# fateshelled/sycl_points

Hardware: AMD Instinct MI355X
Metric: gicp_correspondences_per_sec (higher is better)
Workload: dtype f32

## Files before the change

### include/sycl_points_amd.h

```cpp
#ifndef SYCL_POINTS_AMD_H
#define SYCL_POINTS_AMD_H

#include <stddef.h>
#include <stdint.h>

#ifdef __cplusplus
extern "C" {
#endif

#define SP_OK 0
#define SP_ERR_INVALID_ARGUMENT 1
#define SP_ERR_RUNTIME 2
#define SP_ERR_HIP 3

#define SP_ABI_VERSION 7
int sp_abi_version(void);
void sp_stream_retired(void* stream);
const char* sp_last_error(void);

int sp_device_count(void);
int sp_set_device(int device);


size_t sp_knn_bruteforce_workspace_bytes(size_t nq, size_t nt, size_t k);
// ... 278 lines not shown
typedef struct sp_gicp_target sp_gicp_target;
typedef struct sp_gicp_source sp_gicp_source;
typedef struct sp_gn_params { float lambda, crit_rotation, crit_translation; } sp_gn_params;
enum { SP_SOURCE_ORDER_UNKNOWN = 0, SP_SOURCE_SORT = 1, SP_SOURCE_PRESORTED = 2 };
int sp_gicp_target_create(const sp_grid* grid, const float* tgt_covs, size_t n, void* stream, sp_gicp_target** out);
int sp_gicp_target_update(sp_gicp_target* target, const float* tgt_covs, void* stream);
int sp_gicp_target_create_plain(const sp_grid* grid, const float* tgt_covs, size_t n, void* stream, sp_gicp_target** out);
int sp_gicp_target_certify(sp_gicp_target* target, const float* tgt_covs, void* stream);
int sp_gicp_target_has_certificates(const sp_gicp_target* target);
int sp_gicp_target_prepare(sp_gicp_target* target, const float* tgt_covs, int reg_type, void* stream);
void sp_gicp_target_destroy(sp_gicp_target* target);
int sp_gicp_source_create(size_t n_max, sp_gicp_source** out);
int sp_gicp_source_prepare(sp_gicp_source* source, const sp_gicp_target* target, const float* src_points,
                           const float* src_covs, size_t n, const float* transT, int transT_on_device, int sort_by_cell,
                           void* stream);
void sp_gicp_source_destroy(sp_gicp_source* source);
int sp_gicp_iteration_fused(const sp_gicp_target* target, const sp_gicp_source* source, float* transT,
                            int transT_on_device, const sp_factor_params* params, const sp_gn_params* gn,
                            int32_t* nn_idx_out, float* nn_d2_out, sp_linearized* out, float* delta_out8,
                            void* workspace, size_t workspace_bytes, void* stream);
int sp_gicp_error_prepared(const sp_gicp_target* target, const sp_gicp_source* source, const float* transT_lin_host,
                           const float* transT_trial, int trial_on_device, const sp_factor_params* params,
                           sp_linearized* out, void* workspace, size_t workspace_bytes, void* stream);
int sp_gicp_align_fused(const sp_gicp_target* target, const sp_gicp_source* source, float* transT_device,
                        const sp_factor_params* params, const sp_gn_params* gn, int max_iterations,
                        int32_t* nn_idx_out, float* nn_d2_out, sp_linearized* lin_out, float* delta_out8,
                        uint32_t* iterations_out, void* workspace, size_t workspace_bytes, void* stream);
int sp_gicp_align_step(const sp_gicp_target* target, const sp_gicp_source* source, float* transT_device,
                       const sp_factor_params* params, const sp_gn_params* gn, int k, int rows_all_reduced,
                       int32_t* nn_idx_out, float* nn_d2_out, sp_linearized* lin_out, void* workspace,
// ... 361 lines not shown
```

### sycl_points_amd/_lib.py

```python
import ctypes as C
import os
import subprocess

_HERE = os.path.dirname(os.path.abspath(__file__))
LIB_PATH = os.environ.get("SP_AMD_LIB") or os.path.join(_HERE, "lib", "libsycl_points_amd.so")
CSRC = os.path.join(_HERE, "csrc")

SP_OK, SP_ERR_INVALID_ARGUMENT, SP_ERR_RUNTIME, SP_ERR_HIP = 0, 1, 2, 3
COMM_ID_BYTES = 128


class SpError(RuntimeError):

    def __init__(self, code, msg):
        super().__init__(f"[sycl_points_amd] error {code}: {msg}")
        self.code = code


class Linearized(C.Structure):
    _fields_ = [("H", C.c_float * 36), ("b", C.c_float * 6), ("error", C.c_float), ("inlier", C.c_uint32),
                ("inlier_lo", C.c_float), ("inlier_hi", C.c_float), ("pad", C.c_float * 2)]


class FactorParams(C.Structure):
# ... 250 lines not shown
    "sp_gicp_workspace_bytes": (_sz, [_sz]),
    "sp_gicp_linearize": (_i, [_vp, _vp, _sz, _vp, _vp, _vp, _vp, _vp, _vp, _i, C.POINTER(FactorParams), _vp, _vp, _sz, _vp]),
    "sp_gicp_error": (_i, [_vp, _vp, _sz, _vp, _vp, _vp, _vp, _vp, _vp, _i, C.POINTER(FactorParams), _vp, _vp, _sz, _vp]),
    "sp_icp_robust_weights": (_i, [_vp, _vp, _sz, _vp, _vp, _vp, _vp, _vp, _vp, _i, C.POINTER(FactorParams), _vp, _vp]),
    "sp_genz_counts": (_i, [_vp, _vp, _vp, _sz, _f, _f, _vp, _vp]),
    "sp_gicp_target_create": (_i, [_vp, _vp, _sz, _vp, C.POINTER(_vp)]),
    "sp_gicp_target_create_plain": (_i, [_vp, _vp, _sz, _vp, C.POINTER(_vp)]),
    "sp_gicp_target_certify": (_i, [_vp, _vp, _vp]),
    "sp_gicp_target_has_certificates": (_i, [_vp]),
    "sp_gicp_target_update": (_i, [_vp, _vp, _vp]),
    "sp_gicp_target_prepare": (_i, [_vp, _vp, _i, _vp]),
    "sp_gicp_error_prepared": (_i, [_vp, _vp, _vp, _vp, _i, C.POINTER(FactorParams), _vp, _vp, _sz, _vp]),
    "sp_gicp_target_destroy": (None, [_vp]),
    "sp_gicp_source_create": (_i, [_sz, C.POINTER(_vp)]),
    "sp_gicp_source_prepare": (_i, [_vp, _vp, _vp, _vp, _sz, _vp, _i, _i, _vp]),
    "sp_gicp_source_destroy": (None, [_vp]),
    "sp_gicp_iteration_fused": (_i, [_vp, _vp, _vp, _i, C.POINTER(FactorParams), _vp, _vp, _vp, _vp, _vp, _vp, _sz, _vp]),
    "sp_gicp_align_optimize": (_i, [_vp, _vp, _vp, C.POINTER(FactorParams), C.POINTER(OptParams), C.POINTER(C.c_float), _i, _vp, _vp,
                                    _sz, _vp]),
    "sp_gicp_source_set_persistent": (_i, [_vp, _i]),
    "sp_gicp_source_set_wave_per_point": (_i, [_vp, _i]),
    "sp_gicp_align_batch_workspace_bytes": (_sz, [_sz, _sz]),
    "sp_gicp_align_batch": (_i, [_vp, _vp, _vp, _vp, _sz, C.POINTER(FactorParams), C.POINTER(OptParams), C.POINTER(C.c_float), _i, _vp,
                                 _vp, _sz, _vp]),
    "sp_align_best_host": (_i, [_vp, _sz, C.POINTER(_sz)]),
    "sp_opt_stepper_create": (_i, [C.POINTER(OptParams), _vp, C.POINTER(C.c_float), _i, C.POINTER(_vp)]),
    "sp_opt_stepper_destroy": (None, [_vp]),
    "sp_opt_stepper_next": (_i, [_vp, C.POINTER(OptRequest)]),
    "sp_opt_stepper_linearized": (_i, [_vp, C.POINTER(Linearized)]),
    "sp_opt_stepper_trial": (_i, [_vp, _f, C.c_uint32, C.POINTER(C.c_float)]),
# ... 96 lines not shown
    "sp_pc2_pack": (_i, [_vp, _vp, _vp, _vp, _sz, C.c_double, _vp, _vp]),
    "sp_enhanced_reflectivity_workspace_bytes": (_sz, [_sz]),
    "sp_enhanced_reflectivity": (_i, [_vp, _vp, _sz, _vp, C.c_uint32, C.c_int32, _i, C.c_int32, _vp, _f, _f, _vp, _vp]),
}


INTERNAL_SIGNATURES = {
    "sp_internal_source_option": (_i, [_vp, _i, _i]),
    "sp_internal_grid_option": (_i, [_vp, _i, _i]),
    "sp_internal_bvh_option": (_i, [_vp, _i, _i]),
    "sp_internal_bvh_walk_counts": (_i, [_vp, C.POINTER(C.c_uint32), C.POINTER(C.c_uint32)]),
    "sp_internal_grid_small_build": (_i, [_i]),
    "sp_internal_align_searched_log": (_vp, [_vp, _vp]),
    "sp_internal_source_tile_floats": (_sz, [_vp]),
    "sp_internal_source_tiles_copy": (_i, [_vp, _vp, _sz, _i, _vp]),
    "sp_internal_radix_sort_workspace_bytes": (_sz, [_sz]),
    "sp_internal_radix_sort_u32": (_i, [_vp, _vp, _vp, _vp, _sz, C.c_uint, _vp, _sz, _vp, _vp]),
    "sp_internal_radix_sort_u32_ex": (_i, [_vp, _vp, _vp, _vp, _sz, C.c_uint, C.c_uint, _i, _vp, _sz, _vp, _vp]),
    "sp_internal_radix_first_pass": (None, [_sz, C.c_uint, _vp]),
    "sp_internal_radix_sort_u64": (_i, [_vp, _vp, _vp, _vp, _sz, C.c_uint, _vp, _sz, _vp, _vp]),
    "sp_internal_exclusive_scan_workspace_bytes": (_sz, [_sz]),
    "sp_internal_exclusive_scan_u32": (_i, [_vp, _vp, _sz, _vp, _vp, _sz, _vp]),
    "sp_internal_atan2f_host": (None, [_vp, _vp, _sz, _vp]),
    "sp_internal_fps": (_i, [_i, _vp, _sz, _sz, C.c_uint32, _vp, _vp, _vp, _vp, _sz, _vp]),
    "sp_internal_eigen3": (_i, [_vp, _sz, _vp, _vp, _vp]),
    "sp_internal_inverse3": (_i, [_vp, _sz, _vp, _vp]),
    "sp_internal_bbox": (_i, [_vp, _sz, C.c_uint, _vp, _vp]),
    "sp_internal_morton_keys": (_i, [_vp, _sz, _vp, _vp, _i, _vp, _vp]),
    "sp_internal_sorted_insert": (_i, [_i, _i, _i, _vp, _vp, _sz, _sz, _vp, _vp, _vp]),
    "sp_internal_block_reduce": (_i, [_vp, _vp, _i, _i, _vp, _vp]),
# ... 45 lines not shown
```

### sycl_points_amd/api.py

```python
import ctypes as C
import enum
import sys
import weakref
from dataclasses import dataclass, field

import numpy as np
import torch

from . import _lib
from ._lib import (DegenerateRegParams, FactorParams, GnParams, Linearized, MapPriorParams, MapPriorState, SpError,
                   check)

_SOURCE_ORDER = {False: 0, True: 1, 0: 0, 1: 1, 2: 2, "presorted": 2}
REG = {"POINT_TO_POINT": 0, "POINT_TO_PLANE": 1, "POINT_TO_DISTRIBUTION": 2, "GICP": 3, "GENZ": 4}
LOSS = {"NONE": 0, "HUBER": 1, "TUKEY": 2, "CAUCHY": 3, "GEMAN_MCCLURE": 4}
FLT_MAX = float(np.finfo(np.float32).max)


def _stream():
    return C.c_void_p(torch.cuda.current_stream().cuda_stream)


def _ptr(t):
    return None if t is None else C.c_void_p(t.data_ptr())
# ... 1422 lines not shown
        except Exception:
            pass


class PreparedSource:

    def __init__(self, n_max):
        h = C.c_void_p()
        check(_lib.lib().sp_gicp_source_create(n_max, C.byref(h)))
        self._h = h
        self.n_max = n_max

    def _set_option(self, name, value):
        check(_lib.lib().sp_internal_source_option(self._h, _lib.INTERNAL_OPTION[name], int(value)))

    def prepare(self, prepared_target, source, transT=None, sort_by_cell=True):
        p2d = getattr(prepared_target, "reg_type", "GICP") == "POINT_TO_DISTRIBUTION"
        if not source.has_cov() and not p2d:
            raise SpError(2, "[Registration::validate_params] Covariance matrices of source and target must be "
                             "pre-computed before performing GICP matching.")
        tp, on_dev, keep = _trans_arg(transT)
        check(_lib.lib().sp_gicp_source_prepare(self._h, prepared_target._h, _ptr(source.points),
                                                _ptr(source.covs if source.has_cov() else None),
                                                source.size(), tp, on_dev, _SOURCE_ORDER[sort_by_cell], _stream()))
        self.n = source.size()

    def __del__(self):
        try:
            if self._h:
                _lib.lib().sp_gicp_source_destroy(self._h)
                self._h = None
        except Exception:
            pass


@dataclass
class RegistrationParams:
    reg_type: str = "GICP"
    max_correspondence_distance: float = 2.0
# ... 1162 lines not shown
```

### sycl_points_amd/csrc/registration.hip

```cpp
#include <algorithm>
#include <mutex>

#include "registration_device.h"
#include "sp_wave_solve.h"
#include "sp_cov_normal.h"

namespace sp {
namespace {


struct PointTerm {
    float H[6][6];
    float b[6];
    float sq;
    float residual_norm;
    float genz_weight;
};

__device__ __forceinline__ void se3_jacobian(const Rigid& T, float px, float py, float pz, float J[3][6]) {
#pragma unroll
    for (int i = 0; i < 3; ++i) {
        const float r0 = T.R[i][0], r1 = T.R[i][1], r2 = T.R[i][2];
        J[i][0] = chain3(r0, 0.0f, r1, pz, r2, -py);
        J[i][1] = chain3(r0, -pz, r1, 0.0f, r2, px);
// ... 733 lines not shown
        fused_point<LOSS, FAST_NN, P2D, kSeedSearches, kNegCert, true>(P, T, i, acc, cnt, searched, &head, use_head);
        use_head = false;
        head.x = head.y = head.z = 0.0f;
        head.r0 = head.r1 = head.r2 = make_float4(0.0f, 0.0f, 0.0f, 0.0f);
    }
    if constexpr (!SHARDED) {
        block_reduce_store<kAcc - 1, kAlignBlock>(acc, cnt, partials + (size_t)blockIdx.x * kPartial, false, searched);
    } else if (A.mode == ALIGN_ROWS) {
        block_reduce_store<kAcc - 1, kAlignBlock>(acc, cnt, partials + (size_t)blockIdx.x * kPartial, true, searched);
    } else {
        block_reduce_store<kAcc - 1, kAlignBlock, true>(acc, cnt, partials + (size_t)blockIdx.x * kPartial, false, searched);
        align_tail(A, partials);
    }
}

struct PersistArgs {
    AlignWs ws;
    unsigned* tickets;
    const float* T_init;
    float lambda, crit_rot, crit_trans;
    sp_linearized* lin_out;
    float* T_out;
    float* delta_out8;
    uint32_t* iterations_out;
    int max_iterations;
    int k_begin;
    int cache_valid_later;
    unsigned long long budget;
};
template <int LOSS, bool FAST_NN, bool P2D = false>
// ... 462 lines not shown
    if (e == hipSuccess) e = hipMalloc(&s->qcert2, std::min<size_t>(n, 2048) * sizeof(float4));
    if (e == hipSuccess) e = hipMalloc(&s->opt_rows, sp::kOptRowsBytes);
    if (e == hipSuccess) e = hipMemset(s->opt_rows, 0, sp::kOptRowsBytes);
    if (e == hipSuccess) e = hipMalloc(&s->keys_in, n * 4);
    if (e == hipSuccess) e = hipMalloc(&s->keys_out, n * 4);
    if (e == hipSuccess) e = hipMalloc(&s->vals_in, n * 4);
    if (e == hipSuccess) e = hipMalloc(&s->sort_tmp, s->sort_tmp_bytes ? s->sort_tmp_bytes : 16);
    if (e != hipSuccess) {
        sp_set_error(hipGetErrorString(e));
        sp_gicp_source_destroy(s);
        return SP_ERR_HIP;
    }
    *out = s;
    return SP_OK;
}
extern "C" int sp_gicp_source_prepare(sp_gicp_source* s, const sp_gicp_target* target, const float* src_points,
                                      const float* src_covs, size_t n, const float* transT, int transT_on_device,
                                      int sort_by_cell, void* stream) {
    using namespace sp;
    if (!s || !target) return SP_ERR_INVALID_ARGUMENT;
    if (n > s->n_max) {
        sp_set_error("[sp_gicp_source_prepare] more points than the object was created for");
        return SP_ERR_INVALID_ARGUMENT;
    }
    if (!src_covs && n && target->reg_type == SP_REG_GICP) {
        sp_set_error("[Registration::validate_params] Covariance matrices of source and target must be pre-computed "
                     "before performing GICP matching.");
        return SP_ERR_RUNTIME;
    }
    s->n = n;
    s->sorted = sort_by_cell != 0;
    if (n == 0) return SP_OK;
    hipStream_t st = as_stream(stream);
    const float4* pts = reinterpret_cast<const float4*>(src_points);
    const unsigned nb = div_up(n, kBlock);
// ... 3 lines not shown
        unsigned end_bit = 1;
        while ((1ull << end_bit) <= target->grid->ncells && end_bit < 32) ++end_bit;
        const unsigned begin_bit = end_bit > 16 ? end_bit - 16 : 0;
        bool in_b = false;
        if (radix_sort_pairs_u32(s->keys_in, s->keys_out, s->vals_in, s->perm, n, end_bit, s->sort_tmp, s->sort_tmp_bytes, &in_b,
                                 st, begin_bit) != SP_OK) {
            sp_set_error("[Registration] radix sort of the source failed");
            return SP_ERR_HIP;
        }
        if (!in_b) { unsigned* t = s->perm; s->perm = s->vals_in; s->vals_in = t; }
    }
    s->cache_valid = false;
    s->qcert_valid = false;
    s->cache_target = target;
    s->cache_version = target->version;
    prepare_source_kernel<<<nb, kBlock, 0, st>>>(pts, target->reg_type == SP_REG_GICP ? reinterpret_cast<const float4*>(src_covs) : nullptr,
                                                 s->perm, sort_by_cell != SP_SOURCE_SORT, (unsigned)n, s->tiles);
    return launch_status();
}



extern "C" int sp_gicp_iteration_fused(const sp_gicp_target* target, const sp_gicp_source* source, float* transT,
                                       int transT_on_device, const sp_factor_params* params, const sp_gn_params* gn,
                                       int32_t* nn_idx_out, float* nn_d2_out, sp_linearized* out, float* delta_out8,
                                       void* workspace, size_t workspace_bytes, void* stream) {
    using namespace sp;
    hipStream_t st = as_stream(stream);
    if (!target || !source || !params || !out) return SP_ERR_INVALID_ARGUMENT;
    if (const int rc = check_prepared_reg(target, params); rc != SP_OK) return rc;
    if (gn && !transT_on_device) {
        sp_set_error("[sp_gicp_iteration_fused] the fused Gauss-Newton update needs the pose on the device");
        return SP_ERR_INVALID_ARGUMENT;
    }
    const size_t n = source->n;
    if (n == 0) return zero_async(out, sizeof(sp_linearized), st);
    if (const int rc = check_workspace(workspace, workspace_bytes, n); rc != SP_OK) return rc;
    target->note(st);
    const FusedParams P = make_fused_params(target, source, params, transT, transT_on_device, nn_idx_out, nn_d2_out);
    const bool fills_cache = P.ccache != nullptr && (source->opt_stage_mask & 1);
    const unsigned grid = reduce_grid(n);
    float* partials = static_cast<float*>(workspace);
    const int rc = with_variant(params->robust_type, source_fast_nn(source), params->reg_type == SP_REG_POINT_TO_DISTRIBUTION,
                                [&](auto L, auto FAST_NN, auto P2D) {
        if (source->opt_stage_mask & 1)
            gicp_fused_kernel<L, FAST_NN, P2D><<<grid, kBlock, 0, st>>>(P, partials);
        return SP_OK;
    });
    if (rc != SP_OK) return rc;
    if (fills_cache) { source->cache_valid = true; source->qcert_valid = false; }
    GnArgs ga{nullptr, 0.0f, 0.0f, 0.0f, nullptr};
    if (gn) ga = GnArgs{transT, gn->lambda, gn->crit_rotation, gn->crit_translation, delta_out8};
    if (source->opt_stage_mask & 2) final_reduce_kernel<<<1, kFinalThreads, 0, st>>>(partials, grid, kAcc - 1, out, ga);
// ... 50 lines not shown
                                      const float* transT_trial, int trial_on_device, const sp_factor_params* params,
                                      sp_linearized* out, void* workspace, size_t workspace_bytes, void* stream) {
    using namespace sp;
    hipStream_t st = as_stream(stream);
    if (!target || !source || !params || !out || !transT_lin_host) return SP_ERR_INVALID_ARGUMENT;
    if (const int rc = check_prepared_reg(target, params); rc != SP_OK) return rc;
    const size_t n = source->n;
    if (n == 0) return zero_async(out, sizeof(sp_linearized), st);
    if (const int rc = check_workspace(workspace, workspace_bytes, n); rc != SP_OK) return rc;
    if (!source->cache_valid || source->cache_target != target || source->cache_version != target->version) {
        sp_set_error("[sp_gicp_error_prepared] no frozen correspondences: linearise first (sp_gicp_iteration_fused / "
                     "sp_gicp_align_*) with this target");
        return SP_ERR_RUNTIME;
    }
    target->note(st);
    const FusedParams P = make_fused_params(target, source, params, transT_trial, trial_on_device, nullptr, nullptr);
    Mat4Arg TL;
    for (int i = 0; i < 16; ++i) TL.m[i] = transT_lin_host[i];
    const unsigned grid = reduce_grid(n);
    float* partials = static_cast<float*>(workspace);
    const int rc = with_loss(params->robust_type, [&](auto L) {
        return with_bool<false>(params->reg_type == SP_REG_POINT_TO_DISTRIBUTION, [&](auto P2D) {
            error_prepared_kernel<decltype(L)::value, P2D><<<grid, kBlock, 0, st>>>(P, TL, nullptr, partials);
            return SP_OK;
        });
    });
    if (rc != SP_OK) return rc;
    final_reduce_kernel<<<1, kFinalThreads, 0, st>>>(partials, grid, 1, out, GnArgs{nullptr, 0.0f, 0.0f, 0.0f, nullptr});
    return launch_status();
}
// ... 6 lines not shown
                    const sp_xchg* xchg) {
    hipStream_t st = as_stream(stream);
    if (const int rc = align_check(target, source, params, gn, transT_device, workspace, workspace_bytes); rc != SP_OK) return rc;
    if (k < 0 || rows_all_reduced < 0 || rows_all_reduced > 3 || ((rows_all_reduced == ALIGN_DIRECT) != (xchg != nullptr)))
        return SP_ERR_INVALID_ARGUMENT;
    const size_t n = source->n;
    const AlignWs w = align_ws(workspace);
    const int mode = rows_all_reduced;
    if (k == 0) {
        if (mode != ALIGN_PROLOGUE && zero_async(w.searched_log, kAlignResetBytes, st) != SP_OK) return SP_ERR_HIP;
        if (mode == ALIGN_ROWS &&
            zero_async(w.part[0], 2 * (size_t)kAlignMaxBlocks * kPartial * sizeof(float), st) != SP_OK)
            return SP_ERR_HIP;
    }
    target->note(st);
    const FusedParams P = make_fused_params(target, source, params, transT_device, 1, nn_idx_out, nn_d2_out);
    const bool fills_cache = P.ccache != nullptr && (source->opt_stage_mask & 1);
    const unsigned grid = align_grid(n);
    AlignArgs A = align_args(w, transT_device, gn, k > 0 ? k - 1 : 0, mode, lin_out);
    A.first = k == 0;
    A.prev_rows = w.part[(k + 1) & 1];
    A.k_launch = k;
    A.fan_row_out = w.fan_row[k & 1];
    A.x = xchg_args(xchg);
    float* out = w.part[k & 1];
    const int rc = with_bool<false>(mode != ALIGN_PROLOGUE, [&](auto SHARDED) {
        return with_variant(params->robust_type, source_fast_nn(source), params->reg_type == SP_REG_POINT_TO_DISTRIBUTION,
                            [&](auto L, auto FAST_NN, auto P2D) {
            if (source->opt_stage_mask & 1)
                gicp_align_kernel<L, FAST_NN, P2D, decltype(SHARDED)::value><<<grid, kAlignBlock, 0, st>>>(P, A, out);
            return SP_OK;
        });
    });
    if (rc != SP_OK) return rc;
    if (fills_cache) { source->cache_valid = true; source->qcert_valid = false; }
    return launch_status();
}
}
}

extern "C" int sp_gicp_align_step(const sp_gicp_target* target, const sp_gicp_source* source, float* transT_device,
                                 const sp_factor_params* params, const sp_gn_params* gn, int k, int rows_all_reduced,
                                 int32_t* nn_idx_out, float* nn_d2_out, sp_linearized* lin_out, void* workspace,
                                 size_t workspace_bytes, void* stream) {
    if (rows_all_reduced == sp::ALIGN_DIRECT) return SP_ERR_INVALID_ARGUMENT;
    return sp::align_step_impl(target, source, transT_device, params, gn, k, rows_all_reduced, nn_idx_out, nn_d2_out, lin_out,
                               workspace, workspace_bytes, stream, nullptr);
}
// ... 100 lines not shown
    if (source->opt_persistent == 0 || source->opt_stage_mask != 3) return nullptr;
    if (align_check(target, source, params, gn, T, workspace, workspace_bytes) != SP_OK) return nullptr;
    return persist_acquire(st, align_grid(source->n));
}
int launch_persistent(const sp_gicp_target* target, const sp_gicp_source* source, float* transT_device,
                      const sp_factor_params* params, const sp_gn_params* gn, int k_begin, int max_iterations, int32_t* nn_idx_out,
                      float* nn_d2_out, sp_linearized* lin_out, float* delta_out8, uint32_t* iterations_out, void* workspace,
                      hipStream_t st, PersistGuard* guard) {
    struct Release {
        PersistGuard* g; hipStream_t st;
        ~Release() { persist_release(g, st); }
    } release{guard, st};
    unsigned* const tickets = reinterpret_cast<unsigned*>(static_cast<char*>(workspace) + kTicketOffsetBytes);
    if (zero_async(tickets, kTicketShards * kTicketStride * sizeof(unsigned), st) != SP_OK) return SP_ERR_HIP;
    target->note(st);
    const FusedParams P = make_fused_params(target, source, params, transT_device, 1, nn_idx_out, nn_d2_out);
    PersistArgs A;
    A.ws = align_ws(workspace);
    A.tickets = tickets;
    A.T_init = transT_device;
    A.lambda = gn->lambda; A.crit_rot = gn->crit_rotation; A.crit_trans = gn->crit_translation;
    A.lin_out = lin_out;
    A.T_out = transT_device;
    A.delta_out8 = delta_out8;
    A.iterations_out = iterations_out;
    A.max_iterations = max_iterations;
    A.k_begin = k_begin;
    A.cache_valid_later = (source->opt_reuse && P.ccache != nullptr) ? 1 : 0;
    A.budget = 50ull * 100000ull;
    const unsigned grid = align_grid(source->n);
// ... 83 lines not shown
extern "C" int sp_gicp_source_set_wave_per_point(sp_gicp_source* s, int mode) {
    if (!s || mode < 0 || mode > 2) return SP_ERR_INVALID_ARGUMENT;
    s->opt_wave_query = mode;
    return SP_OK;
}

extern "C" const uint32_t* sp_internal_align_searched_log(void* workspace, size_t* n_entries_out) {
    if (n_entries_out) *n_entries_out = sp::kSearchedLog;
    return workspace ? sp::align_ws(workspace).searched_log : nullptr;
}
extern "C" size_t sp_internal_source_tile_floats(const sp_gicp_source* s) {
    return s ? sp::src_tile_words(s->n_max ? s->n_max : 1) : 0;
}
extern "C" int sp_internal_source_tiles_copy(sp_gicp_source* s, float* device_buffer, size_t n_floats, int to_source, void* stream) {
    if (!s || !device_buffer || n_floats != sp_internal_source_tile_floats(s)) return SP_ERR_INVALID_ARGUMENT;
    const hipError_t e = hipMemcpyAsync(to_source ? s->tiles : device_buffer, to_source ? device_buffer : s->tiles,
                                        n_floats * sizeof(float), hipMemcpyDeviceToDevice, sp::as_stream(stream));
    if (e != hipSuccess) { sp_set_error(hipGetErrorString(e)); return SP_ERR_HIP; }
    return SP_OK;
}
extern "C" int sp_internal_source_option(sp_gicp_source* s, int option, int value) {
    if (!s) return SP_ERR_INVALID_ARGUMENT;
    switch (option) {
        case SP_INTERNAL_FUSED_STAGE_MASK: s->opt_stage_mask = value; return SP_OK;
        case SP_INTERNAL_FUSED_REUSE: s->opt_reuse = value; s->cache_valid = false; return SP_OK;
        case SP_INTERNAL_FUSED_FAST_NN: s->opt_fast_nn = value; return SP_OK;
        case SP_INTERNAL_FUSED_PERSISTENT: s->opt_persistent = value; return SP_OK;
        case SP_INTERNAL_FUSED_PERSISTENT_FROM: s->opt_persistent_from = value < 0 ? 0 : value; return SP_OK;
        case SP_INTERNAL_OPT_WAVE_QUERY: s->opt_wave_query = value; return SP_OK;
        case SP_INTERNAL_OPT_FUSE_TRIALS: s->opt_fuse_trials = value; return SP_OK;
    }
    return SP_ERR_INVALID_ARGUMENT;
// ... 31 lines not shown
```

### sycl_points_amd/csrc/registration_batch.hip

```cpp
#include <cmath>

#include "sp_optimizer.h"

namespace sp {
namespace {

struct BatchArgs {
    float4* rows;
    const float* T_init;
    float* T_out;
    sp_opt_params opt;
    float scales[SP_OPT_MAX_LEVELS];
    int n_levels;
    int reuse;
    sp_align_result* results;
};

__device__ __forceinline__ void batch_after_linearize(OptState& S, const float* tot) {
    unpack_totals(tot, kAcc - 1, &S.slin);
    ++S.ctl.n_lin;
    S.ctl.searched += (unsigned)tot[kAcc];
    opt_after_linearize(S, true);
}
__device__ __forceinline__ void batch_after_trial(OptState& S, const float* tot) {
// ... 110 lines not shown
    }
    const size_t n = source->n;
    if (n == 0 || n > (size_t)SP_ALIGN_BATCH_MAX_POINTS) {
        sp_set_error("[sp_gicp_align_batch] the prepared source must hold 1..SP_ALIGN_BATCH_MAX_POINTS points");
        return SP_ERR_INVALID_ARGUMENT;
    }
    if (!workspace || workspace_bytes < batch_rows_bytes(n, batch)) {
        sp_set_error("[sp_gicp_align_batch] workspace too small (sp_gicp_align_batch_workspace_bytes)");
        return SP_ERR_INVALID_ARGUMENT;
    }
    if (!sp_gicp_target_has_certificates(target)) {
        sp_set_error("[sp_gicp_align_batch] the prepared target has no reuse certificates (sp_gicp_target_certify)");
        return SP_ERR_INVALID_ARGUMENT;
    }
    target->note(st);
    const FusedParams P = make_fused_params(target, source, params, T_init_device, 1, nullptr, nullptr);
    BatchArgs A;
    A.rows = static_cast<float4*>(workspace);
    A.T_init = T_init_device;
    A.T_out = T_out_device;
    A.opt = *opt;
    for (int l = 0; l < SP_OPT_MAX_LEVELS; ++l) A.scales[l] = robust_scales[l < n_levels ? l : n_levels - 1];
    A.n_levels = n_levels;
    A.reuse = source->opt_reuse ? 1 : 0;
    A.results = results_device;
    const int rc = with_variant(params->robust_type, source_fast_nn(source), params->reg_type == SP_REG_POINT_TO_DISTRIBUTION,
                                [&](auto L, auto FAST_NN, auto P2D) {
        constexpr int loss = L;
        constexpr bool fast_nn = FAST_NN, p2d = P2D;
        return with_bool<false>(n <= 256, [&](auto SMALL) {
// ... 28 lines not shown
```

### sycl_points_amd/csrc/registration_device.h

```cpp
#ifndef SP_REGISTRATION_DEVICE_H
#define SP_REGISTRATION_DEVICE_H

#include "grid_device.h"
#include "radix_sort.h"
#include "sp_linearize.h"
#include "sp_xchg.h"

#include <type_traits>

void sp_set_error(const char* msg);

#include "sp_internal.h"

namespace sp {
namespace {

constexpr int kAcc = 29;
constexpr int kPartial = 32;
constexpr int kMaxBlocks = 1024;

template <bool SC1>
__device__ __forceinline__ void store_row_word(float* p, float v) {
    if (SC1) __hip_atomic_store(p, v, __ATOMIC_RELAXED, __HIP_MEMORY_SCOPE_AGENT);
    else *p = v;
// ... 210 lines not shown
    const float4* tnb;
    GridDesc g;
    unsigned n;
    float max_d2, scale;
    QueryPose pose;
    const unsigned* perm;
    float4* ccache;
    int cache_valid;
    int32_t* nn_idx;
    float* nn_d2;
};

__device__ __forceinline__ const float* src_words(const FusedParams& P, unsigned i) {
    return P.src + ((size_t)(i / kWave) * kSrcTileWords + (i % kWave));
}
__device__ __forceinline__ float4 src_point(const float* __restrict__ w) {
    return make_float4(w[0], w[kWave], w[2 * kWave], 1.0f);
}
__device__ __forceinline__ Sym3 src_cov(const float* __restrict__ w) {
    return Sym3{w[3 * kWave], w[4 * kWave], w[5 * kWave], w[6 * kWave], w[7 * kWave], w[8 * kWave]};
}

template <int LOSS, bool P2D = false, bool ERR_ONLY = false, int NACC = kAcc - 1>
__device__ __forceinline__ void fused_math(const FusedParams& P, const Rigid& T, const float4 s, float qx, float qy,
                                           float qz, const Nearest& nn, const Sym3& Cs, const Sym3& Ct,
                                           float (&acc)[NACC], unsigned& cnt) {
    float t[NACC];
    linearize_terms<LOSS, P2D, ERR_ONLY>(T, s.x, s.y, s.z, qx, qy, qz, nn.x, nn.y, nn.z, Cs, Ct, P.scale, t);
#pragma unroll
    for (int e = 0; e < NACC; ++e) acc[e] += t[e];
// ... 38 lines not shown
    return wide;
}

struct PointHead {
    float x, y, z;
    float4 r0, r1, r2;
};
__device__ __forceinline__ void point_head_load(const FusedParams& P, unsigned i, PointHead& h) {
    const unsigned ic = min(i, max(P.n, 1u) - 1u);
    const float* const sw = src_words(P, ic);
    h.x = sw[0]; h.y = sw[kWave]; h.z = sw[2 * kWave];
    const float4* const row = P.ccache + 3 * (size_t)(P.cache_valid ? ic : 0u);
    h.r0 = row[0]; h.r1 = row[1]; h.r2 = row[2];
}

template <int LOSS, bool FAST_NN, bool P2D = false, bool SEED = true, bool NEG = true, bool PRE = false>
__device__ __forceinline__ void fused_point(const FusedParams& P, const Rigid& T, unsigned i, float (&acc)[kAcc - 1],
                                            unsigned& cnt, unsigned& searched, const PointHead* head = nullptr,
                                            bool use_head = false) {
    const float* const sw = src_words(P, i);
    float4* const row = P.ccache + 3 * (size_t)i;
    float4 s;
    float4 r0 = make_float4(0.0f, 0.0f, 0.0f, 0.0f), r1 = r0, r2 = r0;
    if constexpr (PRE) {
        if (use_head) {
            s = make_float4(head->x, head->y, head->z, 1.0f);
            r0 = head->r0; r1 = head->r1; r2 = head->r2;
        } else {
            s = src_point(sw);
            if (P.cache_valid) { r0 = row[0]; r1 = row[1]; r2 = row[2]; }
        }
    } else {
        s = src_point(sw);
    }
    float qx, qy, qz;
    transform_point(T, s.x, s.y, s.z, qx, qy, qz);
    Nearest nn;
    Sym3 Ct{0.0f, 0.0f, 0.0f, 0.0f, 0.0f, 0.0f};
    bool hit = false;
    bool seeded = false;
    Nearest seed;
    seed.d2 = FLT_MAX; seed.idx = -1; seed.pos = 0; seed.x = seed.y = seed.z = 0.0f;
    if (P.cache_valid) {
        if constexpr (!PRE) { r0 = row[0]; r1 = row[1]; r2 = row[2]; }
        const float d = dist2(qx, qy, qz, r0.x, r0.y, r0.z);
        const unsigned pos = __float_as_uint(r2.w);
        if (certified(P, d, r0.w, qx, qy, qz, pos)) {
            hit = true;
            nn.idx = __float_as_int(r2.z); nn.pos = pos; nn.x = r0.x; nn.y = r0.y; nn.z = r0.z;
            nn.d2 = nn.idx >= 0 ? d : FLT_MAX;
            Ct = Sym3{r1.x, r1.y, r1.z, r1.w, r2.x, r2.y};
        } else if (SEED && __float_as_int(r2.z) >= 0) {
            seed.d2 = d; seed.idx = __float_as_int(r2.z); seed.pos = pos; seed.x = r0.x; seed.y = r0.y; seed.z = r0.z;
            seeded = true;
        }
    }
    if (!hit) {
        ++searched;
        float margin2 = 0.0f;
        const float bound2 = NEG ? search_bound2_margin(P, margin2) : search_bound2(P);
        seeded = seeded && seed.d2 < bound2;
        if (!seeded) { seed.d2 = bound2; seed.idx = -1; seed.pos = 0; seed.x = seed.y = seed.z = 0.0f; }
        if (FAST_NN) {
            nn = grid_nn1_auto(P.tpts, P.tstart, P.g, qx, qy, qz, bound2, &seed);
        } else {
            nn = grid_nn1(P.tpts, P.tstart, P.g, qx, qy, qz, &seed, 0);
        }
        if (NEG) store_correspondence(row, P, nn, Ct, qx, qy, qz, margin2);
        else store_correspondence(row, P, nn, Ct);
    }
    if (P.nn_idx) {
        const unsigned o = P.perm[i];
        P.nn_idx[o] = nn.idx;
        P.nn_d2[o] = nn.d2;
    }
    if (nn.idx < 0 || nn.d2 > P.max_d2) return;
    unsigned i_again = i;
    asm volatile("" : "+v"(i_again));
    const float* const sw_again = src_words(P, i_again);
    const Sym3 Cs = P2D ? Sym3{0.0f, 0.0f, 0.0f, 0.0f, 0.0f, 0.0f} : src_cov(sw_again);
    fused_math<LOSS, P2D>(P, T, src_point(sw_again), qx, qy, qz, nn, Cs, Ct, acc, cnt);
}

#ifdef SP_OPT_TIMING
__device__ unsigned long long g_sp_dbg[24 * 16];
__device__ unsigned g_sp_step;
__device__ unsigned long long g_sp_wg[24 * 8];
#define SP_PSTAMP(k) if (blockIdx.x == 0 && threadIdx.x == 0 && g_sp_step < 24) g_sp_dbg[g_sp_step * 16 + (k)] = wall_clock64()
#else
#define SP_PSTAMP(k)
#endif
template <int LOSS, bool P2D = false>
// ... 263 lines not shown
    size_t n_max = 0, n = 0;
    float* tiles = nullptr;
    unsigned* perm = nullptr;
    float4* ccache = nullptr;
    float4* qcert = nullptr;
    float4* qcert2 = nullptr;
    size_t qcert_points = 0;
    mutable bool qcert_valid = false;
    float4* ccache2 = nullptr;
    unsigned long long* opt_rows = nullptr;
    mutable unsigned opt_epoch = 0;
    mutable bool cache_valid = false;
    const sp_gicp_target* cache_target = nullptr;
    unsigned long long cache_version = 0;
    bool sorted = false;
    int opt_stage_mask = 3;
    int opt_reuse = 2;
    int opt_fast_nn = -1;
    int opt_persistent = 1;
    int opt_persistent_from = 4;
    int opt_fuse_trials = 1;
    int opt_wave_query = 1;
    unsigned *keys_in = nullptr, *keys_out = nullptr, *vals_in = nullptr;
    void* sort_tmp = nullptr;
    size_t sort_tmp_bytes = 0;
};

namespace sp {
namespace {
FusedParams make_fused_params(const sp_gicp_target* target, const sp_gicp_source* source, const sp_factor_params* params,
                              const float* transT, int transT_on_device, int32_t* nn_idx_out, float* nn_d2_out) {
    const size_t n = source->n;
    FusedParams P;
    P.src = source->tiles;
    P.tpts = target->grid->d_pts;
    P.tstart = target->grid->d_start;
    P.tcovp = target->covp;
    P.tnb = source->opt_reuse > 1 ? target->nb : nullptr;
    P.g = grid_desc(target->grid);
    P.n = (unsigned)n;
    P.max_d2 = params->max_correspondence_distance * params->max_correspondence_distance;
    P.scale = params->robust_scale;
    P.pose = query_pose(transT, transT_on_device);
// ... 104 lines not shown
```

### sycl_points_amd/csrc/registration_opt.hip

```cpp
#include <algorithm>

#include "sp_optimizer.h"

namespace sp {
namespace {

struct OptArgs {
    float* part[2];
    unsigned* tickets;
    unsigned long long* trows[2];
    unsigned tag_base;
    float4* rows[2];
    float4* qcert[2];
    int qcert_trusted;
    int fuse;
    const float* T_init;
    float* T_out;
    sp_opt_params opt;
    float scales[SP_OPT_MAX_LEVELS];
    int n_levels;
    int reuse;
    sp_align_result* result;
    unsigned long long budget;
};
// ... 386 lines not shown
    A.rows[1] = source->ccache2;
    const bool margin_certs = waveq && source->opt_reuse != 0 && source->qcert != nullptr && n <= source->qcert_points;
    A.qcert[0] = margin_certs ? source->qcert : nullptr;
    A.qcert[1] = margin_certs ? source->qcert2 : nullptr;
    A.qcert_trusted = (margin_certs && source->qcert_valid && source->cache_valid) ? 1 : 0;
    A.fuse = (waveq && wq_block == 256u && source->ccache2 != nullptr && source->opt_fuse_trials && (!margin_certs || source->qcert2 != nullptr)) ? 1 : 0;
    A.tag_base = 0;
    if (grid > 1 && waveq) {
        if (++source->opt_epoch >= 4096u) {
            if (zero_async(source->opt_rows, kOptRowsBytes, st) != SP_OK) return SP_ERR_HIP;
            source->opt_epoch = 1;
        }
        A.tag_base = source->opt_epoch << 20;
    } else if (grid > 1 && zero_async(A.tickets, kTicketShards * kTicketStride * sizeof(unsigned), st) != SP_OK) return SP_ERR_HIP;
    target->note(st);
    FusedParams P = make_fused_params(target, source, params, transT_device, 1, nullptr, nullptr);
    A.T_init = transT_device;
    A.T_out = transT_device;
    A.opt = *opt;
    for (int l = 0; l < SP_OPT_MAX_LEVELS; ++l) A.scales[l] = robust_scales[l < n_levels ? l : n_levels - 1];
    A.n_levels = n_levels;
    A.reuse = (source->opt_reuse && P.ccache != nullptr) ? 1 : 0;
    A.result = result_device;
    A.budget = 50ull * 100000ull;
    if (P.ccache == nullptr) {
        sp_set_error("[sp_gicp_align_optimize] the prepared target has no reuse certificates");
        return SP_ERR_INVALID_ARGUMENT;
    }
    const int rc = with_variant(params->robust_type, fast, params->reg_type == SP_REG_POINT_TO_DISTRIBUTION,
                                [&](auto L, auto FAST_NN, auto P2D) {
// ... 20 lines not shown
```

### sycl_points_amd/csrc/sp_internal.h

```cpp
#ifndef SP_INTERNAL_H
#define SP_INTERNAL_H

#include "../../include/sycl_points_amd.h"

#ifdef __cplusplus
extern "C" {
#endif

enum {
    SP_INTERNAL_FUSED_STAGE_MASK = 0,
    SP_INTERNAL_FUSED_REUSE = 1,
    SP_INTERNAL_FUSED_FAST_NN = 2,
    SP_INTERNAL_SELF_KNN_MODE = 3,
    SP_INTERNAL_FUSED_PERSISTENT = 4,
    SP_INTERNAL_FUSED_PERSISTENT_FROM = 5,
    SP_INTERNAL_BVH_SELF_HEAP = 6,
    SP_INTERNAL_BVH_SORT_QUERIES = 7,
    SP_INTERNAL_GRID_SORT_QUERIES = 8,
    SP_INTERNAL_OPT_WAVE_QUERY = 9,
    SP_INTERNAL_OPT_FUSE_TRIALS = 10,
    SP_INTERNAL_BVH_WALK_COUNTS = 11
};

int sp_internal_source_option(sp_gicp_source* source, int option, int value);
int sp_internal_grid_option(sp_grid* grid, int option, int value);
int sp_internal_bvh_option(sp_bvh* bvh, int option, int value);
int sp_internal_bvh_walk_counts(const sp_bvh* bvh, uint32_t* handed_on_out, uint32_t* arena_claims_out);
int sp_internal_grid_small_build(int enable);
const uint32_t* sp_internal_align_searched_log(void* workspace, size_t* n_entries_out);
size_t sp_internal_source_tile_floats(const sp_gicp_source* source);
int sp_internal_source_tiles_copy(sp_gicp_source* source, float* device_buffer, size_t n_floats, int to_source, void* stream);
size_t sp_internal_radix_sort_workspace_bytes(size_t n);
int sp_internal_radix_sort_u32(uint32_t* keys_a, uint32_t* keys_b, uint32_t* vals_a, uint32_t* vals_b, size_t n,
                               unsigned bits, void* workspace, size_t workspace_bytes, int* result_in_b_out, void* stream);
int sp_internal_radix_sort_u32_ex(uint32_t* keys_a, uint32_t* keys_b, uint32_t* vals_a, uint32_t* vals_b, size_t n,
                                  unsigned bits, unsigned first_bit, int first_hist_ready, void* workspace,
                                  size_t workspace_bytes, int* result_in_b_out, void* stream);
void sp_internal_radix_first_pass(size_t n, unsigned bits, unsigned* out4);
int sp_internal_radix_sort_u64(uint64_t* keys_a, uint64_t* keys_b, uint32_t* vals_a, uint32_t* vals_b, size_t n,
                               unsigned bits, void* workspace, size_t workspace_bytes, int* result_in_b_out, void* stream);
size_t sp_internal_exclusive_scan_workspace_bytes(size_t n);
int sp_internal_exclusive_scan_u32(const uint32_t* in, uint32_t* out, size_t n, uint32_t* total_out_or_null, void* workspace,
                                   size_t workspace_bytes, void* stream);
void sp_internal_atan2f_host(const float* y, const float* x, size_t n, float* out);
int sp_internal_fps(int form, const float* points, size_t n, size_t sampling_num, uint32_t first_index, uint32_t* order_out,
                    uint8_t* flags_out_opt, float* min_d2_out_opt, void* workspace, size_t workspace_bytes, void* stream);
// ... 16 lines not shown
```

Measured before the change: 34.59 billion.

## Defer source tile preparation and fuse it into first alignment step kernel

Adds a deferred source-prepare entry point that records the source pointers instead of launching prepare_source_kernel. The first align_step prologue launch then runs a new kernel that builds the source tiles (points, regularized covariances, perm) while it computes correspondences, saving one launch and a round-trip through the tile buffer. Every other entry point materializes pending state lazily. The cost is more complexity and a risk of stale-state bugs, and the path only runs when callers pass deferred=True.

```diff
diff --git a/include/sycl_points_amd.h b/include/sycl_points_amd.h
--- a/include/sycl_points_amd.h
+++ b/include/sycl_points_amd.h
@@ -316,6 +316,9 @@
 int sp_gicp_source_prepare(sp_gicp_source* source, const sp_gicp_target* target, const float* src_points,
                            const float* src_covs, size_t n, const float* transT, int transT_on_device, int sort_by_cell,
                            void* stream);
+int sp_gicp_source_prepare_deferred(sp_gicp_source* source, const sp_gicp_target* target, const float* src_points,
+                                    const float* src_covs, size_t n, const float* transT, int transT_on_device,
+                                    int sort_by_cell, void* stream);
 void sp_gicp_source_destroy(sp_gicp_source* source);
 int sp_gicp_iteration_fused(const sp_gicp_target* target, const sp_gicp_source* source, float* transT,
                             int transT_on_device, const sp_factor_params* params, const sp_gn_params* gn,
diff --git a/sycl_points_amd/_lib.py b/sycl_points_amd/_lib.py
--- a/sycl_points_amd/_lib.py
+++ b/sycl_points_amd/_lib.py
@@ -288,6 +288,7 @@
     "sp_gicp_target_destroy": (None, [_vp]),
     "sp_gicp_source_create": (_i, [_sz, C.POINTER(_vp)]),
     "sp_gicp_source_prepare": (_i, [_vp, _vp, _vp, _vp, _sz, _vp, _i, _i, _vp]),
+    "sp_gicp_source_prepare_deferred": (_i, [_vp, _vp, _vp, _vp, _sz, _vp, _i, _i, _vp]),
     "sp_gicp_source_destroy": (None, [_vp]),
     "sp_gicp_iteration_fused": (_i, [_vp, _vp, _vp, _i, C.POINTER(FactorParams), _vp, _vp, _vp, _vp, _vp, _vp, _sz, _vp]),
     "sp_gicp_align_optimize": (_i, [_vp, _vp, _vp, C.POINTER(FactorParams), C.POINTER(OptParams), C.POINTER(C.c_float), _i, _vp, _vp,
@@ -414,6 +415,7 @@
     "sp_internal_align_searched_log": (_vp, [_vp, _vp]),
     "sp_internal_source_tile_floats": (_sz, [_vp]),
     "sp_internal_source_tiles_copy": (_i, [_vp, _vp, _sz, _i, _vp]),
+    "sp_internal_source_perm_copy": (_i, [_vp, _vp, _sz, _vp]),
     "sp_internal_radix_sort_workspace_bytes": (_sz, [_sz]),
     "sp_internal_radix_sort_u32": (_i, [_vp, _vp, _vp, _vp, _sz, C.c_uint, _vp, _sz, _vp, _vp]),
     "sp_internal_radix_sort_u32_ex": (_i, [_vp, _vp, _vp, _vp, _sz, C.c_uint, C.c_uint, _i, _vp, _sz, _vp, _vp]),
diff --git a/sycl_points_amd/api.py b/sycl_points_amd/api.py
--- a/sycl_points_amd/api.py
+++ b/sycl_points_amd/api.py
@@ -1460,15 +1460,16 @@
     def _set_option(self, name, value):
         check(_lib.lib().sp_internal_source_option(self._h, _lib.INTERNAL_OPTION[name], int(value)))
 
-    def prepare(self, prepared_target, source, transT=None, sort_by_cell=True):
+    def prepare(self, prepared_target, source, transT=None, sort_by_cell=True, deferred=False):
         p2d = getattr(prepared_target, "reg_type", "GICP") == "POINT_TO_DISTRIBUTION"
         if not source.has_cov() and not p2d:
             raise SpError(2, "[Registration::validate_params] Covariance matrices of source and target must be "
                              "pre-computed before performing GICP matching.")
         tp, on_dev, keep = _trans_arg(transT)
-        check(_lib.lib().sp_gicp_source_prepare(self._h, prepared_target._h, _ptr(source.points),
-                                                _ptr(source.covs if source.has_cov() else None),
-                                                source.size(), tp, on_dev, _SOURCE_ORDER[sort_by_cell], _stream()))
+        L = _lib.lib()
+        fn = L.sp_gicp_source_prepare_deferred if deferred else L.sp_gicp_source_prepare
+        check(fn(self._h, prepared_target._h, _ptr(source.points), _ptr(source.covs if source.has_cov() else None),
+                 source.size(), tp, on_dev, _SOURCE_ORDER[sort_by_cell], _stream()))
         self.n = source.size()
 
     def __del__(self):
diff --git a/sycl_points_amd/csrc/registration.hip b/sycl_points_amd/csrc/registration.hip
--- a/sycl_points_amd/csrc/registration.hip
+++ b/sycl_points_amd/csrc/registration.hip
@@ -771,6 +771,25 @@
     }
 }
 
+template <int LOSS, bool FAST_NN, bool P2D = false>
+__global__ __launch_bounds__(kAlignBlock) void gicp_align_prep_kernel(FusedParams P, AlignArgs A, PrepArgs R,
+                                                                      float* __restrict__ partials) {
+    __shared__ float sT[16];
+    __shared__ unsigned sflag[2];
+    const unsigned tile = xcd_tile();
+    const unsigned i0 = tile * kAlignBlock + threadIdx.x;
+    if (!align_prologue<false>(A, sT, sflag, [] {})) return;
+    const Rigid T = uniform_pose(sT);
+    float acc[kAcc - 1];
+    unsigned cnt = 0, searched = 0;
+    const unsigned stride = gridDim.x * kAlignBlock;
+#pragma unroll
+    for (int e = 0; e < kAcc - 1; ++e) acc[e] = 0.0f;
+    for (unsigned i = i0; i < P.n; i += stride)
+        fused_point<LOSS, FAST_NN, P2D, kSeedSearches, kNegCert, false, true>(P, T, i, acc, cnt, searched, nullptr, false, &R);
+    block_reduce_store<kAcc - 1, kAlignBlock>(acc, cnt, partials + (size_t)blockIdx.x * kPartial, false, searched);
+}
+
 struct PersistArgs {
     AlignWs ws;
     unsigned* tickets;
@@ -1263,11 +1282,25 @@
     *out = s;
     return SP_OK;
 }
-extern "C" int sp_gicp_source_prepare(sp_gicp_source* s, const sp_gicp_target* target, const float* src_points,
-                                      const float* src_covs, size_t n, const float* transT, int transT_on_device,
-                                      int sort_by_cell, void* stream) {
-    using namespace sp;
+namespace sp {
+namespace {
+int launch_prepare_source(const sp_gicp_source* s, const float* src_points, const float* src_covs, bool identity, hipStream_t st) {
+    prepare_source_kernel<<<div_up(s->n, kBlock), kBlock, 0, st>>>(reinterpret_cast<const float4*>(src_points),
+                                                                  reinterpret_cast<const float4*>(src_covs), s->perm, identity,
+                                                                  (unsigned)s->n, s->tiles);
+    return launch_status();
+}
+}
+int source_materialize(const sp_gicp_source* s, hipStream_t st) {
+    if (!s || !s->pending) return SP_OK;
+    s->pending = false;
+    return launch_prepare_source(s, s->pending_points, s->pending_covs, s->pending_identity, st);
+}
+namespace {
+int source_prepare_impl(sp_gicp_source* s, const sp_gicp_target* target, const float* src_points, const float* src_covs, size_t n,
+                        const float* transT, int transT_on_device, int sort_by_cell, void* stream, bool deferred) {
     if (!s || !target) return SP_ERR_INVALID_ARGUMENT;
+    s->pending = false;
     if (n > s->n_max) {
         sp_set_error("[sp_gicp_source_prepare] more points than the object was created for");
         return SP_ERR_INVALID_ARGUMENT;
@@ -1301,9 +1334,26 @@
     s->qcert_valid = false;
     s->cache_target = target;
     s->cache_version = target->version;
-    prepare_source_kernel<<<nb, kBlock, 0, st>>>(pts, target->reg_type == SP_REG_GICP ? reinterpret_cast<const float4*>(src_covs) : nullptr,
-                                                 s->perm, sort_by_cell != SP_SOURCE_SORT, (unsigned)n, s->tiles);
+    const float* const covs = target->reg_type == SP_REG_GICP ? src_covs : nullptr;
+    if (!deferred) return launch_prepare_source(s, src_points, covs, sort_by_cell != SP_SOURCE_SORT, st);
+    s->pending_points = src_points;
+    s->pending_covs = covs;
+    s->pending_identity = sort_by_cell != SP_SOURCE_SORT;
+    s->pending = true;
     return launch_status();
+}
+}
+}
+
+extern "C" int sp_gicp_source_prepare(sp_gicp_source* s, const sp_gicp_target* target, const float* src_points,
+                                      const float* src_covs, size_t n, const float* transT, int transT_on_device,
+                                      int sort_by_cell, void* stream) {
+    return sp::source_prepare_impl(s, target, src_points, src_covs, n, transT, transT_on_device, sort_by_cell, stream, false);
+}
+extern "C" int sp_gicp_source_prepare_deferred(sp_gicp_source* s, const sp_gicp_target* target, const float* src_points,
+                                               const float* src_covs, size_t n, const float* transT, int transT_on_device,
+                                               int sort_by_cell, void* stream) {
+    return sp::source_prepare_impl(s, target, src_points, src_covs, n, transT, transT_on_device, sort_by_cell, stream, true);
 }
 
 
@@ -1324,6 +1374,7 @@
     if (n == 0) return zero_async(out, sizeof(sp_linearized), st);
     if (const int rc = check_workspace(workspace, workspace_bytes, n); rc != SP_OK) return rc;
     target->note(st);
+    if (const int rc = source_materialize(source, st); rc != SP_OK) return rc;
     const FusedParams P = make_fused_params(target, source, params, transT, transT_on_device, nn_idx_out, nn_d2_out);
     const bool fills_cache = P.ccache != nullptr && (source->opt_stage_mask & 1);
     const unsigned grid = reduce_grid(n);
@@ -1404,6 +1455,7 @@
         return SP_ERR_RUNTIME;
     }
     target->note(st);
+    if (const int rc = source_materialize(source, st); rc != SP_OK) return rc;
     const FusedParams P = make_fused_params(target, source, params, transT_trial, trial_on_device, nullptr, nullptr);
     Mat4Arg TL;
     for (int i = 0; i < 16; ++i) TL.m[i] = transT_lin_host[i];
@@ -1440,6 +1492,10 @@
             return SP_ERR_HIP;
     }
     target->note(st);
+    const bool prep = k == 0 && mode == ALIGN_PROLOGUE && source->pending && !source->cache_valid && (source->opt_stage_mask & 1);
+    if (!prep) {
+        if (const int rc = source_materialize(source, st); rc != SP_OK) return rc;
+    }
     const FusedParams P = make_fused_params(target, source, params, transT_device, 1, nn_idx_out, nn_d2_out);
     const bool fills_cache = P.ccache != nullptr && (source->opt_stage_mask & 1);
     const unsigned grid = align_grid(n);
@@ -1450,14 +1506,26 @@
     A.fan_row_out = w.fan_row[k & 1];
     A.x = xchg_args(xchg);
     float* out = w.part[k & 1];
-    const int rc = with_bool<false>(mode != ALIGN_PROLOGUE, [&](auto SHARDED) {
-        return with_variant(params->robust_type, source_fast_nn(source), params->reg_type == SP_REG_POINT_TO_DISTRIBUTION,
-                            [&](auto L, auto FAST_NN, auto P2D) {
-            if (source->opt_stage_mask & 1)
-                gicp_align_kernel<L, FAST_NN, P2D, decltype(SHARDED)::value><<<grid, kAlignBlock, 0, st>>>(P, A, out);
+    int rc;
+    if (prep) {
+        const PrepArgs R{reinterpret_cast<const float4*>(source->pending_points), reinterpret_cast<const float4*>(source->pending_covs),
+                         source->perm, source->tiles, source->pending_identity ? 1 : 0};
+        rc = with_variant(params->robust_type, source_fast_nn(source), params->reg_type == SP_REG_POINT_TO_DISTRIBUTION,
+                          [&](auto L, auto FAST_NN, auto P2D) {
+            gicp_align_prep_kernel<L, FAST_NN, P2D><<<grid, kAlignBlock, 0, st>>>(P, A, R, out);
             return SP_OK;
         });
-    });
+        if (rc == SP_OK) source->pending = false;
+    } else {
+        rc = with_bool<false>(mode != ALIGN_PROLOGUE, [&](auto SHARDED) {
+            return with_variant(params->robust_type, source_fast_nn(source), params->reg_type == SP_REG_POINT_TO_DISTRIBUTION,
+                                [&](auto L, auto FAST_NN, auto P2D) {
+                if (source->opt_stage_mask & 1)
+                    gicp_align_kernel<L, FAST_NN, P2D, decltype(SHARDED)::value><<<grid, kAlignBlock, 0, st>>>(P, A, out);
+                return SP_OK;
+            });
+        });
+    }
     if (rc != SP_OK) return rc;
     if (fills_cache) { source->cache_valid = true; source->qcert_valid = false; }
     return launch_status();
@@ -1588,6 +1656,7 @@
     unsigned* const tickets = reinterpret_cast<unsigned*>(static_cast<char*>(workspace) + kTicketOffsetBytes);
     if (zero_async(tickets, kTicketShards * kTicketStride * sizeof(unsigned), st) != SP_OK) return SP_ERR_HIP;
     target->note(st);
+    if (const int rc = source_materialize(source, st); rc != SP_OK) return rc;
     const FusedParams P = make_fused_params(target, source, params, transT_device, 1, nn_idx_out, nn_d2_out);
     PersistArgs A;
     A.ws = align_ws(workspace);
@@ -1701,8 +1770,17 @@
 }
 extern "C" int sp_internal_source_tiles_copy(sp_gicp_source* s, float* device_buffer, size_t n_floats, int to_source, void* stream) {
     if (!s || !device_buffer || n_floats != sp_internal_source_tile_floats(s)) return SP_ERR_INVALID_ARGUMENT;
+    if (to_source) s->pending = false;
+    else if (const int rc = sp::source_materialize(s, sp::as_stream(stream)); rc != SP_OK) return rc;
     const hipError_t e = hipMemcpyAsync(to_source ? s->tiles : device_buffer, to_source ? device_buffer : s->tiles,
                                         n_floats * sizeof(float), hipMemcpyDeviceToDevice, sp::as_stream(stream));
+    if (e != hipSuccess) { sp_set_error(hipGetErrorString(e)); return SP_ERR_HIP; }
+    return SP_OK;
+}
+extern "C" int sp_internal_source_perm_copy(sp_gicp_source* s, uint32_t* device_buffer, size_t n, void* stream) {
+    if (!s || !device_buffer || n > (s->n_max ? s->n_max : 1)) return SP_ERR_INVALID_ARGUMENT;
+    if (const int rc = sp::source_materialize(s, sp::as_stream(stream)); rc != SP_OK) return rc;
+    const hipError_t e = hipMemcpyAsync(device_buffer, s->perm, n * sizeof(uint32_t), hipMemcpyDeviceToDevice, sp::as_stream(stream));
     if (e != hipSuccess) { sp_set_error(hipGetErrorString(e)); return SP_ERR_HIP; }
     return SP_OK;
 }
diff --git a/sycl_points_amd/csrc/registration_batch.hip b/sycl_points_amd/csrc/registration_batch.hip
--- a/sycl_points_amd/csrc/registration_batch.hip
+++ b/sycl_points_amd/csrc/registration_batch.hip
@@ -148,6 +148,7 @@
         return SP_ERR_INVALID_ARGUMENT;
     }
     target->note(st);
+    if (const int rc = source_materialize(source, st); rc != SP_OK) return rc;
     const FusedParams P = make_fused_params(target, source, params, T_init_device, 1, nullptr, nullptr);
     BatchArgs A;
     A.rows = static_cast<float4*>(workspace);
diff --git a/sycl_points_amd/csrc/registration_device.h b/sycl_points_amd/csrc/registration_device.h
--- a/sycl_points_amd/csrc/registration_device.h
+++ b/sycl_points_amd/csrc/registration_device.h
@@ -3,6 +3,7 @@
 
 #include "grid_device.h"
 #include "radix_sort.h"
+#include "sp_cov_normal.h"
 #include "sp_linearize.h"
 #include "sp_xchg.h"
 
@@ -248,6 +249,13 @@
 __device__ __forceinline__ const float* src_words(const FusedParams& P, unsigned i) {
     return P.src + ((size_t)(i / kWave) * kSrcTileWords + (i % kWave));
 }
+struct PrepArgs {
+    const float4* pts;
+    const float4* covs;
+    unsigned* perm;
+    float* tiles;
+    int identity;
+};
 __device__ __forceinline__ float4 src_point(const float* __restrict__ w) {
     return make_float4(w[0], w[kWave], w[2 * kWave], 1.0f);
 }
@@ -316,15 +324,25 @@
     h.r0 = row[0]; h.r1 = row[1]; h.r2 = row[2];
 }
 
-template <int LOSS, bool FAST_NN, bool P2D = false, bool SEED = true, bool NEG = true, bool PRE = false>
+template <int LOSS, bool FAST_NN, bool P2D = false, bool SEED = true, bool NEG = true, bool PRE = false, bool PREP = false>
 __device__ __forceinline__ void fused_point(const FusedParams& P, const Rigid& T, unsigned i, float (&acc)[kAcc - 1],
                                             unsigned& cnt, unsigned& searched, const PointHead* head = nullptr,
-                                            bool use_head = false) {
+                                            bool use_head = false, const PrepArgs* prep = nullptr) {
+    static_assert(!(PRE && PREP), "the first launch of an alignment has no prologue to prefetch behind");
     const float* const sw = src_words(P, i);
     float4* const row = P.ccache + 3 * (size_t)i;
     float4 s;
     float4 r0 = make_float4(0.0f, 0.0f, 0.0f, 0.0f), r1 = r0, r2 = r0;
-    if constexpr (PRE) {
+    if constexpr (PREP) {
+        unsigned ih = i;
+        asm volatile("" : "+v"(ih));
+        const unsigned src = prep->identity ? ih : prep->perm[ih];
+        if (prep->identity) prep->perm[ih] = ih;
+        const float4 p = prep->pts[src];
+        float* const w = prep->tiles + ((size_t)(ih / kWave) * kSrcTileWords + (ih % kWave));
+        w[0] = p.x; w[kWave] = p.y; w[2 * kWave] = p.z;
+        s = make_float4(p.x, p.y, p.z, 1.0f);
+    } else if constexpr (PRE) {
         if (use_head) {
             s = make_float4(head->x, head->y, head->z, 1.0f);
             r0 = head->r0; r1 = head->r1; r2 = head->r2;
@@ -341,9 +359,11 @@
     Sym3 Ct{0.0f, 0.0f, 0.0f, 0.0f, 0.0f, 0.0f};
     bool hit = false;
     bool seeded = false;
+    unsigned i_again = i;
+    float4 pp = make_float4(0.0f, 0.0f, 0.0f, 0.0f), pc0 = pp, pc1 = pp, pc2 = pp;
     Nearest seed;
     seed.d2 = FLT_MAX; seed.idx = -1; seed.pos = 0; seed.x = seed.y = seed.z = 0.0f;
-    if (P.cache_valid) {
+    if (!PREP && P.cache_valid) {
         if constexpr (!PRE) { r0 = row[0]; r1 = row[1]; r2 = row[2]; }
         const float d = dist2(qx, qy, qz, r0.x, r0.y, r0.z);
         const unsigned pos = __float_as_uint(r2.w);
@@ -368,6 +388,15 @@
         } else {
             nn = grid_nn1(P.tpts, P.tstart, P.g, qx, qy, qz, &seed, 0);
         }
+        if constexpr (PREP) {
+            asm volatile("" : "+v"(i_again));
+            const unsigned src = prep->identity ? i_again : prep->perm[i_again];
+            pp = prep->pts[src];
+            if constexpr (!P2D) {
+                const float4* const c = prep->covs + 4 * (size_t)src;
+                pc0 = c[0]; pc1 = c[1]; pc2 = c[2];
+            }
+        }
         if (NEG) store_correspondence(row, P, nn, Ct, qx, qy, qz, margin2);
         else store_correspondence(row, P, nn, Ct);
     }
@@ -376,8 +405,22 @@
         P.nn_idx[o] = nn.idx;
         P.nn_d2[o] = nn.d2;
     }
+    if constexpr (PREP) {
+        const float4 p = pp;
+        Sym3 Cs{0.0f, 0.0f, 0.0f, 0.0f, 0.0f, 0.0f};
+        if constexpr (!P2D) {
+            const Mat3 R = plane_regularize(cov_of_columns(pc0, pc1, pc2));
+            Cs = Sym3{R.m[0][0], (R.m[0][1] + R.m[1][0]) * 0.5f, (R.m[0][2] + R.m[2][0]) * 0.5f,
+                      R.m[1][1], (R.m[1][2] + R.m[2][1]) * 0.5f, R.m[2][2]};
+            float* const w = prep->tiles + ((size_t)(i_again / kWave) * kSrcTileWords + (i_again % kWave));
+            w[3 * kWave] = Cs.xx; w[4 * kWave] = Cs.xy; w[5 * kWave] = Cs.xz;
+            w[6 * kWave] = Cs.yy; w[7 * kWave] = Cs.yz; w[8 * kWave] = Cs.zz;
+        }
+        if (nn.idx < 0 || nn.d2 > P.max_d2) return;
+        fused_math<LOSS, P2D>(P, T, make_float4(p.x, p.y, p.z, 1.0f), qx, qy, qz, nn, Cs, Ct, acc, cnt);
+        return;
+    }
     if (nn.idx < 0 || nn.d2 > P.max_d2) return;
-    unsigned i_again = i;
     asm volatile("" : "+v"(i_again));
     const float* const sw_again = src_words(P, i_again);
     const Sym3 Cs = P2D ? Sym3{0.0f, 0.0f, 0.0f, 0.0f, 0.0f, 0.0f} : src_cov(sw_again);
@@ -671,6 +714,10 @@
     const sp_gicp_target* cache_target = nullptr;
     unsigned long long cache_version = 0;
     bool sorted = false;
+    mutable bool pending = false;
+    const float* pending_points = nullptr;
+    const float* pending_covs = nullptr;
+    bool pending_identity = false;
     int opt_stage_mask = 3;
     int opt_reuse = 2;
     int opt_fast_nn = -1;
@@ -684,6 +731,7 @@
 };
 
 namespace sp {
+int source_materialize(const sp_gicp_source* source, hipStream_t stream);
 namespace {
 FusedParams make_fused_params(const sp_gicp_target* target, const sp_gicp_source* source, const sp_factor_params* params,
                               const float* transT, int transT_on_device, int32_t* nn_idx_out, float* nn_d2_out) {
diff --git a/sycl_points_amd/csrc/registration_opt.hip b/sycl_points_amd/csrc/registration_opt.hip
--- a/sycl_points_amd/csrc/registration_opt.hip
+++ b/sycl_points_amd/csrc/registration_opt.hip
@@ -424,6 +424,7 @@
         A.tag_base = source->opt_epoch << 20;
     } else if (grid > 1 && zero_async(A.tickets, kTicketShards * kTicketStride * sizeof(unsigned), st) != SP_OK) return SP_ERR_HIP;
     target->note(st);
+    if (const int rc = source_materialize(source, st); rc != SP_OK) return rc;
     FusedParams P = make_fused_params(target, source, params, transT_device, 1, nullptr, nullptr);
     A.T_init = transT_device;
     A.T_out = transT_device;
diff --git a/sycl_points_amd/csrc/sp_internal.h b/sycl_points_amd/csrc/sp_internal.h
--- a/sycl_points_amd/csrc/sp_internal.h
+++ b/sycl_points_amd/csrc/sp_internal.h
@@ -30,6 +30,7 @@
 const uint32_t* sp_internal_align_searched_log(void* workspace, size_t* n_entries_out);
 size_t sp_internal_source_tile_floats(const sp_gicp_source* source);
 int sp_internal_source_tiles_copy(sp_gicp_source* source, float* device_buffer, size_t n_floats, int to_source, void* stream);
+int sp_internal_source_perm_copy(sp_gicp_source* source, uint32_t* device_buffer, size_t n, void* stream);
 size_t sp_internal_radix_sort_workspace_bytes(size_t n);
 int sp_internal_radix_sort_u32(uint32_t* keys_a, uint32_t* keys_b, uint32_t* vals_a, uint32_t* vals_b, size_t n,
                                unsigned bits, void* workspace, size_t workspace_bytes, int* result_in_b_out, void* stream);
```

Result: slower. 34.18 billion (-1.2%).
